# hanmekim/SceneLib2

Measured on NVIDIA H100. Metric: EKF-SLAM frames/sec @320x240 N=100 feats, higher is better.
Workload: dtype f64 (EKF, scores) + u8/int32 (correlation sums)

## Files before the change

### scenelib2_b200/csrc/sl2_ptx.cuh

```cuda
#pragma once
#include <stdint.h>

__device__ __forceinline__ uint32_t smem_u32(const void *p) { return (uint32_t)__cvta_generic_to_shared(p); }
__device__ __forceinline__ void mbar_init(uint32_t bar, uint32_t count) {
  asm volatile("mbarrier.init.shared::cta.b64 [%0], %1;" ::"r"(bar), "r"(count) : "memory");
}
__device__ __forceinline__ void fence_barrier_init() { asm volatile("fence.mbarrier_init.release.cluster;" ::: "memory"); }
__device__ __forceinline__ void fence_proxy_async() { asm volatile("fence.proxy.async.shared::cta;" ::: "memory"); }
__device__ __forceinline__ void mbar_expect_tx(uint32_t bar, uint32_t bytes) {
  asm volatile("mbarrier.arrive.expect_tx.shared::cta.b64 _, [%0], %1;" ::"r"(bar), "r"(bytes) : "memory");
}
__device__ __forceinline__ bool mbar_try_wait(uint32_t bar, uint32_t phase) {
  uint32_t ok;
  asm volatile(
      "{\n"
      ".reg .pred p;\n"
      "mbarrier.try_wait.parity.shared::cta.b64 p, [%1], %2;\n"
      "selp.u32 %0, 1, 0, p;\n"
      "}\n"
      : "=r"(ok)
      : "r"(bar), "r"(phase)
      : "memory");
  return ok != 0;
}
__device__ __forceinline__ void mbar_wait(uint32_t bar, uint32_t phase) {
  while (!mbar_try_wait(bar, phase)) {
  }
}
```

### scenelib2_b200/csrc/update.cu

```cuda
#include <type_traits>

#include "sl2_context.cuh"
#include "sl2_ptx.cuh"

using namespace sl2;

namespace {

constexpr int UPD_THREADS = 256;
constexpr int UPD_NB = 16;
constexpr int UPD_WS = 20;
constexpr int UPD_DS = 20;
constexpr int UPD_MS = 20;
constexpr int UPD_YS = 68;
constexpr int SOLVE_MAX_WARPS = 8;

__host__ __device__ inline int upd_keven(int kmax) { return (kmax + 1) & ~1; }
__host__ __device__ inline int upd_panw(int kmax) {
  return ((2 * upd_keven(kmax) + 15) & ~15) + 2;
}
__host__ __device__ inline size_t upd_pan_doubles(int kmax) { return (size_t)UPD_NB * upd_panw(kmax); }

__device__ __forceinline__ void dmma884(double &c0, double &c1, double a, double b) {
  asm("mma.sync.aligned.m8n8k4.row.col.f64.f64.f64.f64 {%0,%1}, {%2}, {%3}, {%0,%1};"
// ... 428 lines not shown
  }
  if (D == 8 && kb < nk) {
#pragma unroll
    for (int u = 0; u < 4; ++u) step(b[u]);
  }
#pragma unroll
  for (int q = 0; q < GB; ++q) {
    if (g0 + q < ngroups) {
      const int pc = (g0 + q) * 8 + 2 * lc;
#pragma unroll
      for (int mt = 0; mt < 2; ++mt)
        *reinterpret_cast<double2 *>(pan + (size_t)(mt * 8 + lr) * PW + pc) = make_double2(c[q][2 * mt], c[q][2 * mt + 1]);
    }
  }
}

struct CholSmem {
  double *mult;
  double *dpre;
  int msz;
  double *dg;
  double *Wm;
  double *pan;
  int panw;
};
__host__ __device__ inline size_t chol_smem_doubles(int kmax) {
  const size_t mmax = 2 * upd_keven(kmax);
  return 2 * mmax * UPD_MS + 2 * UPD_NB * CH_DPS + UPD_NB * UPD_DS + UPD_NB * UPD_WS + upd_pan_doubles(kmax);
}
__device__ __forceinline__ CholSmem chol_carve(uint8_t *base, int kmax) {
  CholSmem u;
  const int mmax = 2 * upd_keven(kmax);
  double *p = reinterpret_cast<double *>(base);
  u.msz = mmax * UPD_MS;
  u.mult = p;  p += (size_t)2 * u.msz;
  u.dpre = p;  p += 2 * UPD_NB * CH_DPS;
  u.dg = p;  p += UPD_NB * UPD_DS;
  u.Wm = p;  p += UPD_NB * UPD_WS;
  u.pan = p;
  u.panw = upd_panw(kmax);
  return u;
}

__global__ void __launch_bounds__(UPD_THREADS, 2) upd_chol_kernel(const Sl2Dev d, int stream_lo) {
  extern __shared__ __align__(16) uint8_t smem_raw[];
  pdl_prologue();
  const CholSmem sm = chol_carve(smem_raw, d.kmax);
  const int s = stream_lo + blockIdx.x;
  const int tid = threadIdx.x;
  const int ldg = d.ldg;
  double *__restrict__ G = d.G + (size_t)s * d.mmax * ldg;
  double *__restrict__ Wp = d.Wp + (size_t)s * SL2_MAX_PANELS * 256;
  const int warp = tid >> 5, lane = tid & 31;
  const int lr = lane >> 2, lc = lane & 3;
  __shared__ int s_next;
  const int m = d.upd_m[s];
  if (m == 0) return;
  const int width = m;
  const int PW = sm.panw;
  if (tid == 0) s_next = 1;
  __syncthreads();

  for (int i0 = 0, pidx = 0; i0 < m; i0 += UPD_NB, ++pidx) {
    const int par = pidx & 1;
    const double *__restrict__ mcur = sm.mult + par * sm.msz;
    double *__restrict__ mnext = sm.mult + (par ^ 1) * sm.msz;
    const double *__restrict__ dcur = sm.dpre + par * (UPD_NB * CH_DPS);
    double *__restrict__ dnext = sm.dpre + (par ^ 1) * (UPD_NB * CH_DPS);
    const int nbp = min(UPD_NB, m - i0);
    const int n0 = i0 + UPD_NB;
    const int nbn = n0 < m ? min(UPD_NB, m - n0) : 0;
    const int ngroups = (width - i0 + 7) >> 3;
    const int nk = i0 >> 2;
    const int gb = 4;
    const int nbatch = ngroups > 2 ? (ngroups - 2 + gb - 1) / gb : 0;
    const int nitems = 2 + nbatch;
    bool first = true;
    for (;;) {
      int it;
      if (warp == 0 && first) {
        it = 0;
      } else {
        if (lane == 0) it = atomicAdd(&s_next, 1);
        it = __shfl_sync(0xffffffffu, it, 0);
      }
      if (it >= nitems) break;
      if (it == 0) {
        first = false;
        double c[2][4];
        if (pidx == 0) {
#pragma unroll
          for (int q = 0; q < 2; ++q)
#pragma unroll
            for (int mt = 0; mt < 2; ++mt) {
              const int r = mt * 8 + lr, cc = 8 * q + 2 * lc;
              c[q][2 * mt] = (r < nbp && cc < width) ? G[(size_t)r * ldg + cc] : 0.0;
              c[q][2 * mt + 1] = (r < nbp && cc + 1 < width) ? G[(size_t)r * ldg + cc + 1] : 0.0;
            }
        } else {
#pragma unroll
          for (int q = 0; q < 2; ++q)
#pragma unroll
            for (int mt = 0; mt < 2; ++mt) {
              const double2 v = *reinterpret_cast<const double2 *>(dcur + (mt * 8 + lr) * CH_DPS + 8 * q + 2 * lc);
              c[q][2 * mt] = v.x;
              c[q][2 * mt + 1] = v.y;
            }
#pragma unroll
          for (int u = 0; u < 4; ++u) {
            const int st = nk - 4 + u;
            const double a[2] = {mcur[(4 * st + lc) * UPD_MS + lr], mcur[(4 * st + lc) * UPD_MS + 8 + lr]};
            dmma1684(c[0], a, -a[0]);
            dmma1684(c[1], a, -a[1]);
          }
        }
        {
          double *dg = sm.dg;
#pragma unroll
          for (int q = 0; q < 2; ++q)
#pragma unroll
            for (int mt = 0; mt < 2; ++mt) {
              const int r = mt * 8 + lr, cc = 8 * q + 2 * lc;
              const bool rv = r < nbp;
              *reinterpret_cast<double2 *>(dg + r * UPD_DS + cc) =
                  make_double2((rv && cc < nbp) ? c[q][2 * mt] : (r == cc ? 1.0 : 0.0),
                               (rv && cc + 1 < nbp) ? c[q][2 * mt + 1] : (r == cc + 1 ? 1.0 : 0.0));
            }
          sm.Wm[(lane >> 3) * UPD_WS + 8 + (lane & 7)] = 0.0;
          sm.Wm[(4 + (lane >> 3)) * UPD_WS + 8 + (lane & 7)] = 0.0;
          __syncwarp();
          chol8_inv(dg, sm.Wm, 0, lane);
          __syncwarp();
          {
            double c0 = 0.0, c1 = 0.0;
#pragma unroll
            for (int ks = 0; ks < 2; ++ks)
              dmma884(c0, c1, sm.Wm[lr * UPD_WS + 4 * ks + lc], dg[(4 * ks + lc) * UPD_DS + 8 + lr]);
            __syncwarp();
            *reinterpret_cast<double2 *>(dg + lr * UPD_DS + 8 + 2 * lc) = make_double2(c0, c1);
          }
          __syncwarp();
          {
            double2 cv = *reinterpret_cast<const double2 *>(dg + (8 + lr) * UPD_DS + 8 + 2 * lc);
#pragma unroll
            for (int ks = 0; ks < 2; ++ks) {
              const double v = dg[(4 * ks + lc) * UPD_DS + 8 + lr];
              dmma884(cv.x, cv.y, -v, v);
            }
            *reinterpret_cast<double2 *>(dg + (8 + lr) * UPD_DS + 8 + 2 * lc) = cv;
          }
          __syncwarp();
          chol8_inv(dg, sm.Wm, 8, lane);
          __syncwarp();
          {
            double t0 = 0.0, t1 = 0.0;
#pragma unroll
            for (int ks = 0; ks < 2; ++ks)
              dmma884(t0, t1, dg[(4 * ks + lc) * UPD_DS + 8 + lr], sm.Wm[(4 * ks + lc) * UPD_WS + lr]);
            *reinterpret_cast<double2 *>(dg + (8 + lr) * UPD_DS + 2 * lc) = make_double2(t0, t1);
            __syncwarp();
            double w0 = 0.0, w1 = 0.0;
#pragma unroll
            for (int ks = 0; ks < 2; ++ks)
              dmma884(w0, w1, -sm.Wm[(8 + lr) * UPD_WS + 8 + 4 * ks + lc], dg[(8 + 4 * ks + lc) * UPD_DS + lr]);
            *reinterpret_cast<double2 *>(sm.Wm + (8 + lr) * UPD_WS + 2 * lc) = make_double2(w0, w1);
          }
          __syncwarp();
          if (nbp < UPD_NB)
            for (int e = lane; e < UPD_NB * UPD_NB; e += 32) {
              const int i = e >> 4, j = e & 15;
              if (i >= nbp || j >= nbp) sm.Wm[i * UPD_WS + j] = 0.0;
            }
        }
      } else if (it == 1) {
        if (nbn == 0) continue;
        double c[2][4];
#pragma unroll
        for (int q = 0; q < 2; ++q)
#pragma unroll
          for (int mt = 0; mt < 2; ++mt) {
            const int r = mt * 8 + lr, cc = 8 * q + 2 * lc;
            c[q][2 * mt] = (r < nbn && n0 + cc < width) ? G[(size_t)(n0 + r) * ldg + n0 + cc] : 0.0;
            c[q][2 * mt + 1] = (r < nbn && n0 + cc + 1 < width) ? G[(size_t)(n0 + r) * ldg + n0 + cc + 1] : 0.0;
          }
        double v[CH_D][2];
        const size_t kstride = (size_t)4 * ldg;
        const double *gpre = G + (size_t)lc * ldg + n0 + lr;
        double *mp = mnext + lc * UPD_MS + lr;
        const bool v0 = lr < nbn, v1 = 8 + lr < nbn;
        auto loadv = [&](double *dst) {
          const double x0 = gpre[0], x1 = gpre[8];
          dst[0] = v0 ? -x0 : 0.0;
          dst[1] = v1 ? -x1 : 0.0;
          gpre += kstride;
        };
        auto step = [&](const double *vu) {
          const double a[2] = {vu[0], vu[1]};
          mp[0] = a[0];
          mp[8] = a[1];
          mp += 4 * UPD_MS;
          dmma1684(c[0], a, -a[0]);
          dmma1684(c[1], a, -a[1]);
        };
#pragma unroll
        for (int u = 0; u < CH_D - 1; ++u)
          if (u < nk) loadv(v[u]);
        int kb = 0;
        for (; kb + CH_D <= nk; kb += CH_D) {
#pragma unroll
          for (int u = 0; u < CH_D; ++u) {
            if (kb + u + CH_D - 1 < nk) loadv(v[(u + CH_D - 1) % CH_D]);
            step(v[u]);
          }
        }
#pragma unroll
        for (int q = 0; q < 2; ++q)
#pragma unroll
          for (int mt = 0; mt < 2; ++mt)
            *reinterpret_cast<double2 *>(dnext + (mt * 8 + lr) * CH_DPS + 8 * q + 2 * lc) =
                make_double2(c[q][2 * mt], c[q][2 * mt + 1]);
      } else {
        const int bt = it - 2;
        if (gb == 4) chol_batch<4, 4>(G, ldg, mcur, sm.pan, PW, i0, nbp, nk, ngroups, width, 2 + bt * 4, lr, lc);
        else if (gb == 2) chol_batch<2, 8>(G, ldg, mcur, sm.pan, PW, i0, nbp, nk, ngroups, width, 2 + bt * 2, lr, lc);
        else chol_batch<1, 8>(G, ldg, mcur, sm.pan, PW, i0, nbp, nk, ngroups, width, 2 + bt, lr, lc);
      }
    }
    __syncthreads();
    const int ncol = width - i0;
    for (int e = tid; e < UPD_NB * UPD_NB; e += UPD_THREADS) {
      const int r = e / UPD_NB, cc = e - r * UPD_NB;
      if (r < nbp && cc < nbp && i0 + cc < width)
        G[(size_t)(i0 + r) * ldg + i0 + cc] = (cc >= r) ? sm.dg[r * UPD_DS + cc] : 0.0;
      Wp[(size_t)pidx * 256 + e] = sm.Wm[r * UPD_WS + cc];
      if (r >= nbp || UPD_NB + cc >= ncol) mnext[(i0 + r) * UPD_MS + cc] = 0.0;
    }
    if (tid == 0) s_next = 1;
    {
      double aw[4][2];
#pragma unroll
      for (int mt = 0; mt < 2; ++mt)
#pragma unroll
        for (int ks = 0; ks < 4; ++ks) aw[ks][mt] = sm.Wm[(mt * 8 + lr) * UPD_WS + 4 * ks + lc];
      constexpr int FG = 4;
      for (int gb = 2 + warp; gb * 8 < ncol; gb += FG * (UPD_THREADS / 32)) {
        double c[FG][4];
#pragma unroll
        for (int f = 0; f < FG; ++f) c[f][0] = c[f][1] = c[f][2] = c[f][3] = 0.0;
#pragma unroll
        for (int ks = 0; ks < 4; ++ks) {
          double bv[FG];
#pragma unroll
          for (int f = 0; f < FG; ++f) {
            const int cb = (gb + f * (UPD_THREADS / 32)) * 8 + lr;
            bv[f] = cb < ncol ? sm.pan[(size_t)(4 * ks + lc) * PW + cb] : 0.0;
          }
#pragma unroll
          for (int f = 0; f < FG; ++f) dmma1684(c[f], aw[ks], bv[f]);
        }
#pragma unroll
        for (int f = 0; f < FG; ++f) {
          const int gq = gb + f * (UPD_THREADS / 32);
          const int cc = gq * 8 + 2 * lc;
#pragma unroll
          for (int mt = 0; mt < 2; ++mt) {
            const int r = mt * 8 + lr;
            if (r < nbp && cc < ncol) {
              double *dst = G + (size_t)(i0 + r) * ldg + i0 + cc;
              if (cc + 1 < ncol) *reinterpret_cast<double2 *>(dst) = make_double2(c[f][2 * mt], c[f][2 * mt + 1]);
              else *dst = c[f][2 * mt];
              if (gq < 4) {
                mnext[(i0 + r) * UPD_MS + cc - UPD_NB] = -c[f][2 * mt];
                if (cc + 1 < ncol) mnext[(i0 + r) * UPD_MS + cc + 1 - UPD_NB] = -c[f][2 * mt + 1];
              }
            }
          }
        }
      }
    }
    __syncthreads();
  }
}

__device__ __forceinline__ double c_to_b(const double (&c)[2][2], int ks, int lane) {
  const int lr = lane >> 2, lc = lane & 3;
  const int src = ((4 * (ks & 1) + lc) << 2) | (lr >> 1);
  const double v0 = __shfl_sync(0xffffffffu, c[ks >> 1][0], src);
  const double v1 = __shfl_sync(0xffffffffu, c[ks >> 1][1], src);
  return (lr & 1) ? v1 : v0;
}

template <int NP> struct SolveLayout {
  static constexpr int SPLIT = NP > 13 ? 6 : NP;
  static constexpr int REUSE = NP > 13 ? 4 : NP;
  __host__ __device__ static constexpr int pw(int p) { return 16 * (NP - 1 - p) + 4; }
  __host__ __device__ static constexpr int off_lin(int p0, int p) {
    int o = 0;
    for (int q = p0; q < p; ++q) o += 16 * pw(q);
    return o;
  }
  __host__ __device__ static constexpr int off(int p) { return p < SPLIT ? off_lin(0, p) : off_lin(SPLIT, p); }
  static constexpr int PAN_DOUBLES = off_lin(0, SPLIT < NP - 1 ? SPLIT : NP - 1);
  static constexpr int SMEM_DOUBLES = PAN_DOUBLES + NP * 16 * UPD_WS + NP + (NP & 1) +
                                      2 * SOLVE_MAX_WARPS * 2 * 32 * 2 +
                                      SOLVE_MAX_WARPS * 128;
  static_assert(SPLIT == NP || off_lin(SPLIT, NP - 1) <= off_lin(0, REUSE), "second generation must fit");
};

template <int NP>
__global__ void __launch_bounds__(64 * SOLVE_MAX_WARPS, 1) upd_solve_kernel(const Sl2Dev d, int stream_lo) {
  using L = SolveLayout<NP>;
  extern __shared__ __align__(16) uint8_t smem_raw[];
  pdl_prologue();
  double *pan = reinterpret_cast<double *>(smem_raw);
  double *Wm = pan + L::PAN_DOUBLES;
  const uint32_t bars = smem_u32(Wm + NP * 16 * UPD_WS);
  double2 *xbuf = reinterpret_cast<double2 *>(Wm + NP * 16 * UPD_WS + NP + (NP & 1));
  double *ybuf = reinterpret_cast<double *>(xbuf + 2 * SOLVE_MAX_WARPS * 2 * 32);
  const int s = stream_lo + blockIdx.y;
  const int m = d.upd_m[s];
  if (m == 0) return;
  const int tid = threadIdx.x, nthr = blockDim.x;
  const int ngrp = nthr >> 6;
  const int warp = tid >> 5, lane = tid & 31, lr = lane >> 2, lc = lane & 3;
  const int g = warp % ngrp, rho = warp / ngrp;
  const int n = SL2_NXV + 3 * d.nfeat[s];
  const int ncols = n + 1;
  if (blockIdx.x * ngrp * 8 >= ncols) return;
  const int ldg = d.ldg;
  double *__restrict__ G = d.G + (size_t)s * d.mmax * ldg;
  const double *__restrict__ Wp = d.Wp + (size_t)s * SL2_MAX_PANELS * 256;
  const int m8 = (m + 7) & ~7;
  const bool full = L::SPLIT == NP && m8 >= 16 * NP - 8;
  const int zend = full ? 16 * NP : m8;

  if (tid == 0) {
    for (int p = 0; p < NP; ++p) mbar_init(bars + 8 * p, 1);
    fence_barrier_init();
    fence_proxy_async();
  }
  auto zero_pads = [&](int plo, int phi) {
    for (int e = tid; e < (phi - plo) * 16; e += nthr) {
      const int p = plo + (e >> 4), r = e & 15;
      const int cfirst = 16 * p + 16;
      if (16 * p < m)
        for (int c = max(m, cfirst); c < zend; ++c) pan[L::off(p) + r * L::pw(p) + (c - cfirst)] = 0.0;
    }
  };
  zero_pads(0, L::SPLIT);
  __syncthreads();
  auto request = [&](int p) {
    if (16 * p < m) {
      const int cfirst = 16 * p + 16;
      const int nrow = min(16, m - 16 * p);
      const uint32_t ubytes = m > cfirst ? (uint32_t)(m - cfirst) * 8u : 0u;
      const uint32_t bar = bars + 8 * p;
      if (lane == 0) mbar_expect_tx(bar, (uint32_t)nrow * ubytes + 16u * 128u);
      __syncwarp();
      if (lane < 16) {
        if (lane < nrow && ubytes)
          bulk_g2s(pan + L::off(p) + lane * L::pw(p), G + (size_t)(16 * p + lane) * ldg + cfirst, ubytes, bar);
      } else {
        bulk_g2s(Wm + ((size_t)p * 16 + (lane - 16)) * UPD_WS, Wp + (size_t)p * 256 + (lane - 16) * 16, 128u, bar);
      }
    }
  };
  if (warp == 0) {
#pragma unroll 1
    for (int p = 0; p < L::SPLIT; ++p) request(p);
  }

  int xpar = 0;
  auto solve_group = [&](auto full_c, const int grp) {
    constexpr bool FULL = decltype(full_c)::value;
    const int c0 = 8 * grp;
    const bool wact = c0 < ncols;
    const int cc = c0 + 2 * lc;
    const int cval = wact ? min(2, ncols - cc) : 0;
    double *gcol = G + m + cc;
    double acc[(NP + 1) & ~1][2];
    {
      const int ccn = cc + 8 * (int)(gridDim.x * ngrp);
      if (L::SPLIT >= NP && ccn < ncols) {
#pragma unroll
        for (int t = 0; t < NP; ++t) {
          const int row = 8 * (2 * t + rho) + lr;
          if (row < m) asm volatile("prefetch.global.L2 [%0];" ::"l"(G + m + ccn + (size_t)row * ldg));
        }
      }
    }
#pragma unroll
    for (int t = 0; t < ((NP + 1) & ~1); ++t) {
      const int row = 8 * (2 * t + rho) + lr;
      acc[t][0] = acc[t][1] = 0.0;
      if (row < m) {
        if (cval >= 2) {
          const double2 v = *reinterpret_cast<const double2 *>(gcol + (size_t)row * ldg);
          acc[t][0] = v.x;
          acc[t][1] = v.y;
        } else if (cval == 1) {
          acc[t][0] = gcol[(size_t)row * ldg];
        }
      }
    }

#pragma unroll
    for (int p = 0; p < NP; ++p) {
      if (FULL || 16 * p < m) {
        if (L::SPLIT < NP && p == L::REUSE) {
          __syncthreads();
          zero_pads(L::SPLIT, NP);
          __syncthreads();
          if (warp == 0) {
            fence_proxy_async();
#pragma unroll 1
            for (int q = L::SPLIT; q < NP; ++q) request(q);
          }
        }
        if (!wact) continue;
        xpar ^= 1;
        double2 *xb = xbuf + ((size_t)(xpar * ngrp + g) * 2) * 32;
        xb[rho * 32 + lane] = make_double2(acc[p][0], acc[p][1]);
        asm volatile("bar.sync %0, 64;" ::"r"(1 + g) : "memory");
        const double2 other = xb[(rho ^ 1) * 32 + lane];
        const double cp2[2][2] = {{rho ? other.x : acc[p][0], rho ? other.y : acc[p][1]},
                                  {rho ? acc[p][0] : other.x, rho ? acc[p][1] : other.y}};
        mbar_wait(bars + 8 * p, 0);
        const double *pb = pan + L::off(p);
        const int PW = L::pw(p);
        const double *wb = Wm + (size_t)p * 16 * UPD_WS;
        double cb[4];
#pragma unroll
        for (int ks = 0; ks < 4; ++ks) cb[ks] = c_to_b(cp2, ks, lane);
        double d0 = 0.0, d1 = 0.0;
#pragma unroll
        for (int ks = 0; ks < 4; ++ks) dmma884(d0, d1, wb[(8 * rho + lr) * UPD_WS + 4 * ks + lc], cb[ks]);
        {
          const int row = 16 * p + 8 * rho + lr;
          if (row < m) {
            if (cval >= 2) *reinterpret_cast<double2 *>(gcol + (size_t)row * ldg) = make_double2(d0, d1);
            else if (cval == 1) gcol[(size_t)row * ldg] = d0;
          }
        }
        if (p + 1 < NP) {
          double *yg = ybuf + (size_t)g * 128;
          *reinterpret_cast<double2 *>(yg + (8 * rho + lr) * 8 + 2 * lc) = make_double2(d0, d1);
          asm volatile("bar.sync %0, 64;" ::"r"(1 + g) : "memory");
          double yb[4];
#pragma unroll
          for (int ks = 0; ks < 4; ++ks) yb[ks] = -yg[(4 * ks + lc) * 8 + lr];
          const double *pbr = pb + 8 * rho + lr;
#pragma unroll
          for (int ks = 0; ks < 4; ++ks) {
#pragma unroll
            for (int t = (p + 1) & ~1; t < NP; t += 2) {
              const bool has[2] = {t > p && (FULL || 8 * (2 * t + rho) < m),
                                   t + 1 < NP && (FULL || 8 * (2 * t + 2 + rho) < m)};
              if (has[0] || has[1]) {
                double a[2];
#pragma unroll
                for (int h = 0; h < 2; ++h) a[h] = has[h] ? pbr[(4 * ks + lc) * PW + 16 * (t + h - p - 1)] : 0.0;
                double c[4] = {acc[t][0], acc[t][1], acc[t + 1][0], acc[t + 1][1]};
                dmma1684(c, a, yb[ks]);
                acc[t][0] = c[0];
                acc[t][1] = c[1];
                acc[t + 1][0] = c[2];
                acc[t + 1][1] = c[3];
              }
            }
          }
        }
      }
    }
  };
  for (int grp = blockIdx.x * ngrp + g; L::SPLIT < NP ? grp == (int)(blockIdx.x * ngrp + g) : 8 * grp < ncols;
       grp += gridDim.x * ngrp) {
    if (L::SPLIT == NP && full) solve_group(std::true_type{}, grp);
    else solve_group(std::false_type{}, grp);
  }
}

constexpr int SYRK_THREADS = 128;
template <int KC, int ST>
__global__ void __launch_bounds__(SYRK_THREADS, 3) upd_syrk_kernel(const Sl2Dev d, int stream_lo) {
  constexpr int STAGE = 2 * KC * UPD_YS;
  constexpr int NW = SYRK_THREADS / 32;
  extern __shared__ __align__(16) uint8_t smem_raw[];
  double *stage_buf = reinterpret_cast<double *>(smem_raw);
  pdl_prologue();
  const int s = stream_lo + blockIdx.y;
  const int m = d.upd_m[s];
  if (m == 0) return;
  const int n = SL2_NXV + 3 * d.nfeat[s];
  int tb = 0;
  const int t = blockIdx.x;
  while ((tb + 1) * (tb + 2) / 2 <= t) ++tb;
  const int ta = t - tb * (tb + 1) / 2;
  if (tb * 64 >= n + 1) return;
  const int tid = threadIdx.x, warp = tid >> 5, lane = tid & 31, lr = lane >> 2, lc = lane & 3;
  const int wa = (warp & 1) * 32, wb = (warp >> 1) * 32;
  const int ld = d.ld, ldg = d.ldg;
  double *__restrict__ P = d.P + (size_t)s * ld * ld;
  double *__restrict__ x = d.x + (size_t)s * ld;
  const double *__restrict__ G = d.G + (size_t)s * d.mmax * ldg;
  const bool diag = ta == tb;
  const int bi0 = wa >> 3, bj0 = wb >> 3;
  unsigned cmask = 0xFFFFu, mmask = 0xFFFFu;
  if (diag) {
    cmask = mmask = 0u;
#pragma unroll
    for (int bi = 0; bi < 4; ++bi)
#pragma unroll
      for (int bj = 0; bj < 4; ++bj) {
        if (bi0 + bi <= bj0 + bj) cmask |= 1u << (4 * bi + bj);
        if (bi0 + bi < bj0 + bj) mmask |= 1u << (4 * bi + bj);
      }
  }
  const bool skip = cmask == 0u;
  if (!skip) {
#pragma unroll
    for (int i = 0; i < 4; ++i) {
      const int a = ta * 64 + wa + i * 8, bq = tb * 64 + wb + lane;
      if (a < n && bq < n) asm volatile("prefetch.global.L2 [%0];" ::"l"(P + a + (size_t)ld * bq));
    }
  }
  const int kr = m, lim = m + n + 1;
  const int nchunk = (kr + KC - 1) / KC;
  const int cA = m + ta * 64 + 2 * lane, cB = m + tb * 64 + 2 * lane;
  const int bytesA = cA + 1 < lim ? 16 : (cA < lim ? 8 : 0);
  const int bytesB = cB + 1 < lim ? 16 : (cB < lim ? 8 : 0);
  const double *srcA = G + (bytesA ? cA : 0);
  const double *srcB = G + (bytesB ? cB : 0);
  const double *pa = srcA + (size_t)warp * ldg, *pb = srcB + (size_t)warp * ldg;
  const uint32_t sdst = smem_u32(stage_buf + 2 * lane + warp * UPD_YS);
  const size_t rstep = (size_t)NW * ldg;
  auto stage = [&](int chunk) {
    const uint32_t dd = sdst + (uint32_t)(chunk % ST) * (STAGE * 8);
    if ((chunk + 1) * KC <= kr) {
#pragma unroll
      for (int j = 0; j < KC / NW; ++j) {
        asm volatile("cp.async.cg.shared.global [%0], [%1], 16, %2;" ::"r"(dd + j * NW * UPD_YS * 8),
                     "l"(pa + j * rstep), "r"(bytesA)
                     : "memory");
        if (!diag)
          asm volatile("cp.async.cg.shared.global [%0], [%1], 16, %2;" ::"r"(dd + (KC + j * NW) * UPD_YS * 8),
                       "l"(pb + j * rstep), "r"(bytesB)
                       : "memory");
      }
    } else {
#pragma unroll
      for (int j = 0; j < KC / NW; ++j) {
        const bool kv = chunk * KC + warp + NW * j < kr;
        asm volatile("cp.async.cg.shared.global [%0], [%1], 16, %2;" ::"r"(dd + j * NW * UPD_YS * 8),
                     "l"(kv ? pa + j * rstep : srcA), "r"(kv ? bytesA : 0)
                     : "memory");
        if (!diag)
          asm volatile("cp.async.cg.shared.global [%0], [%1], 16, %2;" ::"r"(dd + (KC + j * NW) * UPD_YS * 8),
                       "l"(kv ? pb + j * rstep : srcB), "r"(kv ? bytesB : 0)
                       : "memory");
      }
    }
    pa += (size_t)KC * ldg;
    pb += (size_t)KC * ldg;
  };
  double acc[2][4][4];
#pragma unroll
  for (int i = 0; i < 2; ++i)
#pragma unroll
    for (int j = 0; j < 4; ++j)
#pragma unroll
      for (int e = 0; e < 4; ++e) acc[i][j][e] = 0.0;
#pragma unroll
  for (int c = 0; c < ST - 1; ++c) {
    if (c < nchunk) stage(c);
    cp_async_commit();
  }
  for (int ch = 0; ch < nchunk; ++ch) {
    cp_async_wait<ST - 2>();
    __syncthreads();
    if (ch + ST - 1 < nchunk) stage(ch + ST - 1);
    cp_async_commit();
    if (!skip) {
      const double *Ya = stage_buf + (size_t)(ch % ST) * STAGE;
      const double *Yb = diag ? Ya : Ya + KC * UPD_YS;
      const int krem = kr - ch * KC;
      auto chunk = [&](auto diag_c) {
        constexpr bool DIAG = decltype(diag_c)::value;
        auto kstep = [&](int kk) {
          double a[2][4], b[4][2];
#pragma unroll
          for (int i = 0; i < 2; ++i)
#pragma unroll
            for (int e = 0; e < 4; ++e)
              a[i][e] = Ya[(kk + lc + 4 * (e >> 1)) * UPD_YS + wa + 16 * i + 8 * (e & 1) + lr];
#pragma unroll
          for (int j = 0; j < 4; ++j)
#pragma unroll
            for (int e = 0; e < 2; ++e) b[j][e] = Yb[(kk + lc + 4 * e) * UPD_YS + wb + j * 8 + lr];
#pragma unroll
          for (int i = 0; i < 2; ++i)
#pragma unroll
            for (int j = 0; j < 4; ++j)
              if (!DIAG || 2 * i <= j) dmma1688(acc[i][j], a[i], b[j]);
        };
        if (krem >= KC) {
#pragma unroll
          for (int kk = 0; kk < KC; kk += 8) kstep(kk);
        } else {
#pragma unroll 1
          for (int kk = 0; kk < krem; kk += 8) kstep(kk);
        }
      };
      if (cmask == 0xFFFFu) chunk(std::false_type{});
      else chunk(std::true_type{});
    }
  }
  if (skip) return;
#pragma unroll
  for (int bi = 0; bi < 4; ++bi) {
    const int i = bi >> 1, h = bi & 1;
    const int a = ta * 64 + wa + bi * 8 + lr;
    double pold[4][2];
#pragma unroll
    for (int j = 0; j < 4; ++j)
#pragma unroll
      for (int e = 0; e < 2; ++e) {
        const int bq = tb * 64 + wb + j * 8 + 2 * lc + e;
        pold[j][e] = (((cmask >> (4 * bi + j)) & 1u) && a < n && bq < n) ? P[a + (size_t)ld * bq] : 0.0;
      }
#pragma unroll
    for (int j = 0; j < 4; ++j) {
      if (!((cmask >> (4 * bi + j)) & 1u)) continue;
      const int bq = tb * 64 + wb + j * 8 + 2 * lc;
      const double c0 = acc[i][j][2 * h], c1 = acc[i][j][2 * h + 1];
      const double v0 = pold[j][0] - c0, v1 = pold[j][1] - c1;
      if (a < n && bq < n) {
        P[a + (size_t)ld * bq] = v0;
        if (bq + 1 < n) P[a + (size_t)ld * (bq + 1)] = v1;
        if ((mmask >> (4 * bi + j)) & 1u) {
          double *dst = P + bq + (size_t)ld * a;
          if (bq + 1 < n) *reinterpret_cast<double2 *>(dst) = make_double2(v0, v1);
          else *dst = v0;
        }
      }
      if (a < n) {
        if (bq == n) x[a] += c0;
        if (bq + 1 == n) x[a] += c1;
      }
    }
  }
}

__global__ void __launch_bounds__(UPD_THREADS) upd_finish_kernel(const Sl2Dev d, int stream_lo, int staged,
                                                                  int only_normalise) {
  pdl_prologue();
  const int s = stream_lo + blockIdx.x;
  const int tid = threadIdx.x;
  const int nf = d.nfeat[s];
  const int n = SL2_NXV + 3 * nf;
  const int ld = d.ld;
  double *__restrict__ P = d.P + (size_t)s * ld * ld;
  const double *__restrict__ x = d.x + (size_t)s * ld;
  const size_t fb = (size_t)s * d.Nmax;
  const int m = only_normalise ? 0 : d.upd_m[s];
  __shared__ int s_cull;
  if (m > 0 || only_normalise) {
    __shared__ double J4[16];
    if (tid == 0) {
      const rd q[4] = {rd(x[3]), rd(x[4]), rd(x[5]), rd(x[6])};
      const rd qq = q[0] * q[0] + q[1] * q[1] + q[2] * q[2] + q[3] * q[3];
      for (int i = 0; i < 4; ++i)
        for (int j = 0; j < 4; ++j)
          J4[i * 4 + j] = (i == j) ? ((rd(1.0) - q[i] * q[i] / (qq * qq)) / qq).v
                                   : ((-q[i]) * q[j] / (qq * qq * qq)).v;
    }
    __syncthreads();
    for (int j = tid; j < n; j += UPD_THREADS) {
      double v[4], o[4];
      for (int k = 0; k < 4; ++k) v[k] = P[(3 + k) + (size_t)ld * j];
      for (int i = 0; i < 4; ++i) {
        rd a(0.0);
        for (int k = 0; k < 4; ++k) a = a + rd(J4[i * 4 + k]) * rd(v[k]);
        o[i] = a.v;
      }
      for (int k = 0; k < 4; ++k) P[(3 + k) + (size_t)ld * j] = o[k];
    }
    __syncthreads();
    for (int i = tid; i < n; i += UPD_THREADS) {
      if (i < SL2_NXV) {
        double v[4], o[4];
        for (int k = 0; k < 4; ++k) v[k] = P[i + (size_t)ld * (3 + k)];
        for (int c = 0; c < 4; ++c) {
          rd a(0.0);
          for (int k = 0; k < 4; ++k) a = a + rd(v[k]) * rd(J4[c * 4 + k]);
          o[c] = a.v;
        }
        for (int k = 0; k < 4; ++k) P[i + (size_t)ld * (3 + k)] = o[k];
      } else {
        for (int k = 0; k < 4; ++k) P[i + (size_t)ld * (3 + k)] = P[(3 + k) + (size_t)ld * i];
      }
    }
    __syncthreads();
  }
  {
    const int i = tid % 13, j = (tid / 13) % 13;
    const double a = P[i + (size_t)ld * j], b = P[j + (size_t)ld * i];
    const double v = (rd(a) * rd(0.5) + rd(b) * rd(0.5)).v;
    __syncthreads();
    if (tid < 169) P[i + (size_t)ld * j] = v;
    __syncthreads();
  }
  if (!staged && !only_normalise) {
    if (tid == 0) s_cull = 0;
    __syncthreads();
    for (int i = tid; i < nf; i += UPD_THREADS) {
      int att = d.attempted[fb + i], suc = d.successful[fb + i];
      if (d.sel_rank[fb + i] >= 0) {
        att += 1;
        if (d.found[fb + i] == 1) suc += 1;
        d.attempted[fb + i] = att;
        d.successful[fb + i] = suc;
      }
      if (att >= d.min_attempts && (double)suc / (double)att < d.match_fraction) atomicAdd(&s_cull, 1);
    }
    __syncthreads();
    if (tid == 0) d.ncull[s] = s_cull;
  }
}

struct SolveKernel {
  void (*kern)(Sl2Dev, int);
  int np;
  size_t smem;
};
template <int NP>
SolveKernel solve_kernel_np() {
  return {upd_solve_kernel<NP>, NP, SolveLayout<NP>::SMEM_DOUBLES * sizeof(double)};
}
inline SolveKernel solve_kernel(int kmax) {
  const int p = (2 * upd_keven(kmax) + 15) / 16;
  return p <= 4 ? solve_kernel_np<4>()
                : (p <= 7 ? solve_kernel_np<7>()
                          : (p <= 10 ? solve_kernel_np<10>() : (p <= 13 ? solve_kernel_np<13>() : solve_kernel_np<16>())));
}
inline void solve_shape(int Nmax, int &nslab, int &warps) {
  const int ngroups = (SL2_NXV + 3 * Nmax + 1 + 7) / 8;
  nslab = (ngroups + SOLVE_MAX_WARPS - 1) / SOLVE_MAX_WARPS;
  warps = (ngroups + nslab - 1) / nslab;
}
constexpr size_t SYRK_SMEM = (size_t)2 * 2 * 32 * UPD_YS * sizeof(double);

size_t sl2_update_smem_bytes(const Sl2Dev &d) {
  return chol_smem_doubles(d.kmax) * sizeof(double);
}

}

cudaError_t sl2_configure_update(const Sl2Dev &d) {
  const SolveKernel solve = solve_kernel(d.kmax);
  const struct {
    const void *kern;
    size_t smem;
  } opt_in[] = {
      {(const void *)upd_hp_kernel<7>, hp_layout(d.kmax, d.ld, 0).bytes},
      {(const void *)upd_hp_kernel<13>, hp_layout(d.kmax, d.ld, 0).bytes},
      {(const void *)upd_hp2_kernel<7>, hp_layout(d.kmax, d.ld, 7).bytes},
      {(const void *)upd_hp2_kernel<13>, hp_layout(d.kmax, d.ld, 13).bytes},
      {(const void *)upd_chol_kernel, sl2_update_smem_bytes(d)},
      {(const void *)solve.kern, solve.smem},
      {(const void *)upd_syrk_kernel<32, 2>, SYRK_SMEM},
  };
  for (const auto &k : opt_in) {
    const cudaError_t e = cudaFuncSetAttribute(k.kern, cudaFuncAttributeMaxDynamicSharedMemorySize, (int)k.smem);
    if (e != cudaSuccess) return e;
  }
  return cudaSuccess;
}

cudaError_t sl2_launch_update(const Sl2Dev &d, int stream_lo, int stream_cnt, int staged_m,
                              const int *st_feat, const double *st_Hxv, const double *st_Hy,
                              const double *st_R, const double *st_nu, int only_normalise,
// ... 93 lines not shown
```

Before: 233,000.

## Interleave panel rows across warp pair and replace bar.sync with mbarrier handoff

Restructures the blocked triangular solve so each warp of a pair owns alternating 16-row panels (m16n8k4 MMAs) instead of 8-row halves. The warp that owns the next panel forms its Y block and publishes it through per-group mbarriers rather than a 64-thread named barrier. This lets the pair pipeline: one warp applies the current update while the other computes the next diagonal block. The aim is to remove the two bar.sync points per panel and the x-buffer exchange. In return it adds mbarrier phase tracking and slot-reuse waits, which are subtle to get right.

```diff
diff --git a/scenelib2_b200/csrc/sl2_ptx.cuh b/scenelib2_b200/csrc/sl2_ptx.cuh
--- a/scenelib2_b200/csrc/sl2_ptx.cuh
+++ b/scenelib2_b200/csrc/sl2_ptx.cuh
@@ -9,6 +9,9 @@
 __device__ __forceinline__ void fence_proxy_async() { asm volatile("fence.proxy.async.shared::cta;" ::: "memory"); }
 __device__ __forceinline__ void mbar_expect_tx(uint32_t bar, uint32_t bytes) {
   asm volatile("mbarrier.arrive.expect_tx.shared::cta.b64 _, [%0], %1;" ::"r"(bar), "r"(bytes) : "memory");
+}
+__device__ __forceinline__ void mbar_arrive(uint32_t bar) {
+  asm volatile("mbarrier.arrive.shared::cta.b64 _, [%0];" ::"r"(bar) : "memory");
 }
 __device__ __forceinline__ bool mbar_try_wait(uint32_t bar, uint32_t phase) {
   uint32_t ok;
diff --git a/scenelib2_b200/csrc/update.cu b/scenelib2_b200/csrc/update.cu
--- a/scenelib2_b200/csrc/update.cu
+++ b/scenelib2_b200/csrc/update.cu
@@ -754,21 +754,22 @@
   __host__ __device__ static constexpr int off(int p) { return p < SPLIT ? off_lin(0, p) : off_lin(SPLIT, p); }
   static constexpr int PAN_DOUBLES = off_lin(0, SPLIT < NP - 1 ? SPLIT : NP - 1);
   static constexpr int SMEM_DOUBLES = PAN_DOUBLES + NP * 16 * UPD_WS + NP + (NP & 1) +
-                                      2 * SOLVE_MAX_WARPS * 2 * 32 * 2 +
-                                      SOLVE_MAX_WARPS * 128;
+                                      SOLVE_MAX_WARPS * 4 +
+                                      SOLVE_MAX_WARPS * 2 * 128;
   static_assert(SPLIT == NP || off_lin(SPLIT, NP - 1) <= off_lin(0, REUSE), "second generation must fit");
 };
 
 template <int NP>
 __global__ void __launch_bounds__(64 * SOLVE_MAX_WARPS, 1) upd_solve_kernel(const Sl2Dev d, int stream_lo) {
   using L = SolveLayout<NP>;
+  constexpr int NU = (NP + 1) / 2;
   extern __shared__ __align__(16) uint8_t smem_raw[];
   pdl_prologue();
   double *pan = reinterpret_cast<double *>(smem_raw);
   double *Wm = pan + L::PAN_DOUBLES;
   const uint32_t bars = smem_u32(Wm + NP * 16 * UPD_WS);
-  double2 *xbuf = reinterpret_cast<double2 *>(Wm + NP * 16 * UPD_WS + NP + (NP & 1));
-  double *ybuf = reinterpret_cast<double *>(xbuf + 2 * SOLVE_MAX_WARPS * 2 * 32);
+  double *pairbar = Wm + NP * 16 * UPD_WS + NP + (NP & 1);
+  double *ybuf = pairbar + SOLVE_MAX_WARPS * 4;
   const int s = stream_lo + blockIdx.y;
   const int m = d.upd_m[s];
   if (m == 0) return;
@@ -785,9 +786,14 @@
   const int m8 = (m + 7) & ~7;
   const bool full = L::SPLIT == NP && m8 >= 16 * NP - 8;
   const int zend = full ? 16 * NP : m8;
+  const int npan = (m + 15) >> 4;
+  const uint32_t ybar = smem_u32(pairbar + 4 * g);
+  double *yslot = ybuf + (size_t)g * 256;
 
   if (tid == 0) {
     for (int p = 0; p < NP; ++p) mbar_init(bars + 8 * p, 1);
+    for (int i = 0; i < 4 * ngrp; ++i)
+      if ((i & 3) != 3) mbar_init(smem_u32(pairbar + i), 1);
     fence_barrier_init();
     fence_proxy_async();
   }
@@ -822,40 +828,96 @@
     for (int p = 0; p < L::SPLIT; ++p) request(p);
   }
 
-  int xpar = 0;
-  auto solve_group = [&](auto full_c, const int grp) {
+  uint32_t yph = 0;
+  auto solve_group = [&](auto full_c, const int grp, const int gi) {
     constexpr bool FULL = decltype(full_c)::value;
     const int c0 = 8 * grp;
     const bool wact = c0 < ncols;
     const int cc = c0 + 2 * lc;
     const int cval = wact ? min(2, ncols - cc) : 0;
     double *gcol = G + m + cc;
-    double acc[(NP + 1) & ~1][2];
+    double acc[NU][4];
     {
       const int ccn = cc + 8 * (int)(gridDim.x * ngrp);
       if (L::SPLIT >= NP && ccn < ncols) {
 #pragma unroll
-        for (int t = 0; t < NP; ++t) {
-          const int row = 8 * (2 * t + rho) + lr;
-          if (row < m) asm volatile("prefetch.global.L2 [%0];" ::"l"(G + m + ccn + (size_t)row * ldg));
-        }
-      }
-    }
-#pragma unroll
-    for (int t = 0; t < ((NP + 1) & ~1); ++t) {
-      const int row = 8 * (2 * t + rho) + lr;
-      acc[t][0] = acc[t][1] = 0.0;
-      if (row < m) {
-        if (cval >= 2) {
-          const double2 v = *reinterpret_cast<const double2 *>(gcol + (size_t)row * ldg);
-          acc[t][0] = v.x;
-          acc[t][1] = v.y;
-        } else if (cval == 1) {
-          acc[t][0] = gcol[(size_t)row * ldg];
-        }
-      }
-    }
-
+        for (int u = 0; u < NU; ++u)
+#pragma unroll
+          for (int h = 0; h < 2; ++h) {
+            const int row = 16 * (2 * u + rho) + 8 * h + lr;
+            if (row < m) asm volatile("prefetch.global.L2 [%0];" ::"l"(G + m + ccn + row * ldg));
+          }
+      }
+    }
+#pragma unroll
+    for (int u = 0; u < NU; ++u)
+#pragma unroll
+      for (int h = 0; h < 2; ++h) {
+        const int row = 16 * (2 * u + rho) + 8 * h + lr;
+        acc[u][2 * h] = acc[u][2 * h + 1] = 0.0;
+        if (row < m) {
+          if (cval >= 2) {
+            const double2 v = *reinterpret_cast<const double2 *>(gcol + row * ldg);
+            acc[u][2 * h] = v.x;
+            acc[u][2 * h + 1] = v.y;
+          } else if (cval == 1) {
+            acc[u][2 * h] = gcol[row * ldg];
+          }
+        }
+      }
+
+    auto form_y = [&](const int u, const int q) {
+      mbar_wait(bars + 8 * q, 0);
+      const double *wb = Wm + (size_t)q * 16 * UPD_WS;
+      const double cp[2][2] = {{acc[u][0], acc[u][1]}, {acc[u][2], acc[u][3]}};
+      double cb[4];
+#pragma unroll
+      for (int ks = 0; ks < 4; ++ks) cb[ks] = c_to_b(cp, ks, lane);
+      double y[4] = {0.0, 0.0, 0.0, 0.0};
+#pragma unroll
+      for (int ks = 0; ks < 4; ++ks) {
+        const double a[2] = {wb[lr * UPD_WS + 4 * ks + lc], wb[(8 + lr) * UPD_WS + 4 * ks + lc]};
+        dmma1684(y, a, cb[ks]);
+      }
+#pragma unroll
+      for (int h = 0; h < 2; ++h) {
+        const int row = 16 * q + 8 * h + lr;
+        if (row < m) {
+          if (cval >= 2) *reinterpret_cast<double2 *>(gcol + row * ldg) = make_double2(y[2 * h], y[2 * h + 1]);
+          else if (cval == 1) gcol[row * ldg] = y[2 * h];
+        }
+      }
+      if (q + 1 < npan) {
+        if (q == 0 && gi > 0) mbar_wait(ybar + 16, (gi - 1) & 1);
+        double *ys = yslot + 128 * rho;
+        __syncwarp();
+#pragma unroll
+        for (int h = 0; h < 2; ++h)
+          *reinterpret_cast<double2 *>(ys + (8 * h + lr) * 8 + 2 * lc) = make_double2(y[2 * h], y[2 * h + 1]);
+        __syncwarp();
+        if (lane == 0) mbar_arrive(ybar + 8 * rho);
+      }
+    };
+    auto apply = [&](const int u0, const int u1, const int qo, const int p, const double (&yb)[4]) {
+      const double *pa = pan + L::off(p) + lr;
+      const int PW = L::pw(p);
+#pragma unroll
+      for (int ks = 0; ks < 4; ++ks) {
+#pragma unroll
+        for (int u = u0; u < u1; ++u) {
+          const int q = 2 * u + qo;
+          const bool has[2] = {FULL || 16 * q < m, FULL || 16 * q + 8 < m};
+          if (q < NP && has[0]) {
+            double a[2];
+#pragma unroll
+            for (int h = 0; h < 2; ++h) a[h] = has[h] ? pa[(4 * ks + lc) * PW + 16 * (q - p - 1) + 8 * h] : 0.0;
+            dmma1684(acc[u], a, yb[ks]);
+          }
+        }
+      }
+    };
+
+    if (wact && rho == 0) form_y(0, 0);
 #pragma unroll
     for (int p = 0; p < NP; ++p) {
       if (FULL || 16 * p < m) {
@@ -869,66 +931,36 @@
             for (int q = L::SPLIT; q < NP; ++q) request(q);
           }
         }
-        if (!wact) continue;
-        xpar ^= 1;
-        double2 *xb = xbuf + ((size_t)(xpar * ngrp + g) * 2) * 32;
-        xb[rho * 32 + lane] = make_double2(acc[p][0], acc[p][1]);
-        asm volatile("bar.sync %0, 64;" ::"r"(1 + g) : "memory");
-        const double2 other = xb[(rho ^ 1) * 32 + lane];
-        const double cp2[2][2] = {{rho ? other.x : acc[p][0], rho ? other.y : acc[p][1]},
-                                  {rho ? acc[p][0] : other.x, rho ? acc[p][1] : other.y}};
+        if (!wact || p + 1 >= NP || !(FULL || p + 1 < npan)) continue;
+        const int k = p & 1;
+        if (rho != k) {
+          mbar_wait(ybar + 8 * k, yph);
+          yph ^= 1;
+        }
+        double yb[4];
+#pragma unroll
+        for (int ks = 0; ks < 4; ++ks) yb[ks] = -yslot[128 * k + (4 * ks + lc) * 8 + lr];
+        if (rho == 1 && k == 0 && p + 4 > npan) {
+          __syncwarp();
+          if (lane == 0) mbar_arrive(ybar + 16);
+        }
         mbar_wait(bars + 8 * p, 0);
-        const double *pb = pan + L::off(p);
-        const int PW = L::pw(p);
-        const double *wb = Wm + (size_t)p * 16 * UPD_WS;
-        double cb[4];
-#pragma unroll
-        for (int ks = 0; ks < 4; ++ks) cb[ks] = c_to_b(cp2, ks, lane);
-        double d0 = 0.0, d1 = 0.0;
-#pragma unroll
-        for (int ks = 0; ks < 4; ++ks) dmma884(d0, d1, wb[(8 * rho + lr) * UPD_WS + 4 * ks + lc], cb[ks]);
-        {
-          const int row = 16 * p + 8 * rho + lr;
-          if (row < m) {
-            if (cval >= 2) *reinterpret_cast<double2 *>(gcol + (size_t)row * ldg) = make_double2(d0, d1);
-            else if (cval == 1) gcol[(size_t)row * ldg] = d0;
-          }
-        }
-        if (p + 1 < NP) {
-          double *yg = ybuf + (size_t)g * 128;
-          *reinterpret_cast<double2 *>(yg + (8 * rho + lr) * 8 + 2 * lc) = make_double2(d0, d1);
-          asm volatile("bar.sync %0, 64;" ::"r"(1 + g) : "memory");
-          double yb[4];
-#pragma unroll
-          for (int ks = 0; ks < 4; ++ks) yb[ks] = -yg[(4 * ks + lc) * 8 + lr];
-          const double *pbr = pb + 8 * rho + lr;
-#pragma unroll
-          for (int ks = 0; ks < 4; ++ks) {
-#pragma unroll
-            for (int t = (p + 1) & ~1; t < NP; t += 2) {
-              const bool has[2] = {t > p && (FULL || 8 * (2 * t + rho) < m),
-                                   t + 1 < NP && (FULL || 8 * (2 * t + 2 + rho) < m)};
-              if (has[0] || has[1]) {
-                double a[2];
-#pragma unroll
-                for (int h = 0; h < 2; ++h) a[h] = has[h] ? pbr[(4 * ks + lc) * PW + 16 * (t + h - p - 1)] : 0.0;
-                double c[4] = {acc[t][0], acc[t][1], acc[t + 1][0], acc[t + 1][1]};
-                dmma1684(c, a, yb[ks]);
-                acc[t][0] = c[0];
-                acc[t][1] = c[1];
-                acc[t + 1][0] = c[2];
-                acc[t + 1][1] = c[3];
-              }
-            }
-          }
+        if (rho == k) {
+          apply((p >> 1) + 1, NU, k, p, yb);
+        } else {
+          const int u1 = (p + 1) >> 1;
+          apply(u1, u1 + 1, 1 - k, p, yb);
+          form_y(u1, p + 1);
+          apply(u1 + 1, NU, 1 - k, p, yb);
         }
       }
     }
   };
+  int gi = 0;
   for (int grp = blockIdx.x * ngrp + g; L::SPLIT < NP ? grp == (int)(blockIdx.x * ngrp + g) : 8 * grp < ncols;
-       grp += gridDim.x * ngrp) {
-    if (L::SPLIT == NP && full) solve_group(std::true_type{}, grp);
-    else solve_group(std::false_type{}, grp);
+       grp += gridDim.x * ngrp, ++gi) {
+    if (L::SPLIT == NP && full) solve_group(std::true_type{}, grp, gi);
+    else solve_group(std::false_type{}, grp, gi);
   }
 }
 
```

Result: faster. 236,300 (median of 6 runs) (+1.4%).
